# rrwick/Badread

Hardware: NVIDIA H100
Metric: simulated Gbases/sec (higher is better)
Workload: dtype u8/int32 (+f64 identity estimate)

## Files before the change

badread_b200/csrc/bb_api.cu:

```cuda
#include <cuda_runtime.h>
#include <dlfcn.h>
#include <unistd.h>

#include <algorithm>
#include <atomic>
#include <cstdio>
#include <cstdlib>
#include <cstring>
#include <numeric>
#include <string>
#include <thread>
#include <vector>

#include "bb_kernels.cuh"
#include "bb_launch.h"

namespace {

struct DevBuf {
    void *p = nullptr;
    size_t cap = 0;
    bool borrowed = false;
    void borrow(const DevBuf &o) { release(); p = o.p; cap = o.cap; borrowed = true; }
    cudaError_t ensure(size_t bytes) {
        if (bytes <= cap && !borrowed) return cudaSuccess;
        if (borrowed) { p = nullptr; cap = 0; borrowed = false; }
        if (p) { cudaFree(p); p = nullptr; cap = 0; }
        size_t want = bytes + bytes / 8 + 256;
        cudaError_t e = cudaMalloc(&p, want);
        if (e == cudaSuccess) cap = want;
        return e;
    }
    void release() { if (p && !borrowed) cudaFree(p); p = nullptr; cap = 0; borrowed = false; }
    template <typename T> T *as() const { return reinterpret_cast<T *>(p); }
};

constexpr int BB_MAX_ROUNDS = 15;

const char *kStageNames[BB_N_STAGES] = {"build_fragments", "error_loop", "scan", "join", "final_align", "qscores",
                                        "compact", "total"};

}

struct bb_ctx {
    int device = 0;
    int sm_count = 0;
    uint64_t seed = 0;
    cudaStream_t stream = nullptr, stream2 = nullptr;
    cudaStream_t side[2][3] = {};
    cudaEvent_t ev_side[2][3] = {}, ev_level[2] = {};
    cudaEvent_t ev_fork = nullptr, ev_join = nullptr;
    std::string err;
    int64_t launches = 0;

    DevBuf ref; int64_t ref_len = 0;
    bool have_em = false, have_qm = false;
    BBErrorModelDev em{}; DevBuf em_k2r, em_rowoff, em_cum, em_flags, em_slots, em_pool, em_rowinfo;
    BBQScoreModelDev qm{}; DevBuf qm_hkeys, qm_hvals, qm_lkeys, qm_lpool, qm_rowoff, qm_scores, qm_cum;

    int n_reads = 0;
    bool uploaded = false, ran = false;
    std::vector<BBReadDev> h_reads;
    std::vector<int32_t> h_inlen;
    std::vector<double> h_target;
    int64_t frag_total = 0, out_total = 0;
    int64_t seq_cap = 0, out_cap = 0, speq_cap = 0;
    int64_t log_total = 0, wres_total = 0;
    int max_len = 0;
    double slack = 1.25;
    int n_rounds = 3;
    int n_levels = 0;
    int extra_levels = 0;
    bool lr_worst = false;
    int lr_cap = 0;
    struct RunInfo { BBScanOut scan; int counters[256]; int qcount[2][32]; } *h_info = nullptr;
    std::vector<BBReadDev> h_res;
    bool finished = false;
    bool reran = false;
    int n_reruns = 0;
    uint32_t rerun_reasons = 0;
    DevBuf d_scan;
    void *nccl_comm = nullptr;
    DevBuf d_red;
    cudaEvent_t ev_scan = nullptr;
    DevBuf d_read_index, d_seg_off, d_segs, d_lit, d_target, d_order, d_reads;
    int n_lane_reads = 0, n_long_reads = 0;
    std::vector<int> h_order;
    DevBuf d_kidx, d_frag, d_state, d_seq, d_ops, d_dcnt, d_qual, d_out_seq, d_out_qual, d_counter, d_fpeq, d_speq, d_fallback;
    int64_t fpeq_total = 0;

    int n_warps = 0;
    BBScratchPool pool{}, pool_lean{};
    DevBuf s_hist, s_hbuf, s_lr, s_stack, s_tbuf, s_peq, s_ltbuf, s_leafhist, s_lr_lean, s_wckpt, s_lanehist;
    DevBuf d_ctime, d_chlog, d_wres, d_wtasks, d_wfallback, d_active;
    DevBuf p_q, p_t, p_ops, p_dcnt, p_out, p_qual;
    int lane8_cols = 4096;
    int pair_ctas = 1;
    bool head_worker = true;
    bool is_head = false;
    bool lpt_order = true;
    int ring_t = 4;
    bool lowmem = false;
    bool use_quad = false;
    int grid_div_env = 0;
    int grid_div = 1;
    struct QueueBufs { DevBuf node[BBQ_NODE_CLASSES][2], leaf[2], count; } qbuf[2];


    cudaEvent_t ev[BB_N_STAGES + 1] = {};
    float stage_ms[BB_N_STAGES] = {};

    std::vector<bb_ctx *> kids;
    int n_split = 1;
    std::vector<std::vector<int32_t>> part;
    std::vector<int64_t> part_base;
    cudaEvent_t ev_t0 = nullptr, ev_t1 = nullptr;

    bool trace = false;
    struct Mark { const char *name; int stream; cudaEvent_t ev; };
    std::vector<Mark> marks;
    std::vector<cudaEvent_t> mark_pool;
    size_t mark_used = 0;
};

static void mark(bb_ctx *ctx, cudaStream_t st, const char *name) {
    if (!ctx->trace) return;
    if (ctx->mark_used == ctx->mark_pool.size()) {
        cudaEvent_t e;
        if (cudaEventCreate(&e) != cudaSuccess) return;
        ctx->mark_pool.push_back(e);
    }
    cudaEvent_t e = ctx->mark_pool[ctx->mark_used++];
    cudaEventRecord(e, st);
    int id = st == ctx->stream ? 0 : st == ctx->stream2 ? 1 : -1;
    for (int p = 0; p < 2 && id < 0; p++)
        for (int x = 0; x < 3; x++)
            if (st == ctx->side[p][x]) id = 2 + 4 * p + x;
    ctx->marks.push_back(bb_ctx::Mark{name, id < 0 ? 0 : id, e});
}

static thread_local std::string g_create_error;

namespace {
struct ConnectionsDefault {
    ConnectionsDefault() { setenv("CUDA_DEVICE_MAX_CONNECTIONS", "32", 0); }
} g_connections_default;
}

#define BB_CUDA(ctx, call)                                                                                   \
    do {                                                                                                     \
        cudaError_t e_ = (call);                                                                             \
        if (e_ != cudaSuccess) {                                                                             \
            (ctx)->err = std::string(#call) + ": " + cudaGetErrorString(e_);                                 \
            return BB_ERR_CUDA;                                                                              \
        }                                                                                                    \
    } while (0)

static int set_err(bb_ctx *ctx, int code, const std::string &msg) {
    if (ctx) ctx->err = msg;
    return code;
}

extern "C" const char *bb_version(void) { return "badread_b200 0.1.0 (sm_90a)"; }

extern "C" const char *bb_last_error(const bb_ctx *ctx) { return ctx ? ctx->err.c_str() : g_create_error.c_str(); }

extern "C" const char *bb_stage_name(int stage) {
    return (stage >= 0 && stage < BB_N_STAGES) ? kStageNames[stage] : "";
}

extern "C" int64_t bb_launch_count(const bb_ctx *ctx) {
    if (!ctx) return 0;
    int64_t total = ctx->launches;
    for (const bb_ctx *kid : ctx->kids) total += kid->launches;
    return total;
}

static int create_worker(bb_ctx **out, int device, uint64_t seed, bool high_priority = false) {
    if (!out) return BB_ERR_ARG;
    *out = nullptr;
    int n_dev = 0;
    cudaError_t e = cudaGetDeviceCount(&n_dev);
    if (e != cudaSuccess || n_dev <= 0) {
        g_create_error = std::string("no CUDA device available: ") + cudaGetErrorString(e) +
                         " (badread_b200 has no CPU path)";
        return BB_ERR_CUDA;
    }
    if (device < 0 || device >= n_dev) { g_create_error = "invalid device ordinal"; return BB_ERR_ARG; }
    e = cudaSetDevice(device);
    if (e != cudaSuccess) { g_create_error = cudaGetErrorString(e); return BB_ERR_CUDA; }
    bb_ctx *ctx = new bb_ctx();
    ctx->device = device;
    ctx->seed = seed;
    cudaDeviceProp prop;
    e = cudaGetDeviceProperties(&prop, device);
    if (e != cudaSuccess) { g_create_error = cudaGetErrorString(e); delete ctx; return BB_ERR_CUDA; }
    ctx->sm_count = prop.multiProcessorCount;
    int prio_lo = 0, prio_hi = 0;
    cudaDeviceGetStreamPriorityRange(&prio_lo, &prio_hi);
    const int prio = high_priority ? prio_hi : prio_lo;
    e = cudaStreamCreateWithPriority(&ctx->stream, cudaStreamNonBlocking, prio);
    if (e != cudaSuccess) { g_create_error = cudaGetErrorString(e); delete ctx; return BB_ERR_CUDA; }
    for (auto &ev : ctx->ev) cudaEventCreate(&ev);
    cudaStreamCreateWithPriority(&ctx->stream2, cudaStreamNonBlocking, prio);
    cudaEventCreateWithFlags(&ctx->ev_fork, cudaEventDisableTiming);
    cudaEventCreateWithFlags(&ctx->ev_join, cudaEventDisableTiming);
    cudaEventCreateWithFlags(&ctx->ev_scan, cudaEventDisableTiming);
    for (int p = 0; p < 2; p++) {
        cudaEventCreateWithFlags(&ctx->ev_level[p], cudaEventDisableTiming);
        for (int x = 0; x < 3; x++) {
            cudaStreamCreateWithPriority(&ctx->side[p][x], cudaStreamNonBlocking, prio);
            cudaEventCreateWithFlags(&ctx->ev_side[p][x], cudaEventDisableTiming);
        }
    }
    if (cudaHostAlloc((void **)&ctx->h_info, sizeof(bb_ctx::RunInfo), cudaHostAllocPortable) != cudaSuccess) {
        g_create_error = "cudaHostAlloc failed"; delete ctx; return BB_ERR_CUDA;
    }
    uint8_t comp[256];
    std::memset(comp, 'N', sizeof(comp));
    const char *from = "ATGCatgcRYSWKMBVDHNryswkmbvdhn.-?";
    const char *to = "TACGtacgYRSWMKVBHDNyrswmkvbhdn.-?";
    for (int i = 0; from[i]; i++) comp[(uint8_t)from[i]] = (uint8_t)to[i];
    e = cudaMemcpyToSymbol(bb_c_comp, comp, 256);
    if (e != cudaSuccess) { g_create_error = cudaGetErrorString(e); delete ctx; return BB_ERR_CUDA; }
    e = bbl_node_pair_init();
    if (e == cudaSuccess) e = bbl_node_quad_init();
    if (e == cudaSuccess) e = bbl_window_lane_init();
    if (e == cudaSuccess) e = bbl_leaf_lane_init();
    if (e != cudaSuccess) { g_create_error = cudaGetErrorString(e); delete ctx; return BB_ERR_CUDA; }
    ctx->n_warps = ctx->sm_count * 4 * BB_WARPS_PER_CTA;
    if (const char *e = std::getenv("BADREAD_B200_TRACE")) ctx->trace = (e[0] == '1');
    if (const char *e = std::getenv("BADREAD_B200_LANE8_COLS")) ctx->lane8_cols = std::atoi(e);
    if (const char *e = std::getenv("BADREAD_B200_PAIR_CTAS")) ctx->pair_ctas = (e[0] == '2') ? 2 : 1;
    if (const char *e = std::getenv("BADREAD_B200_HEAD_WORKER")) ctx->head_worker = (e[0] != '0');
    if (const char *e = std::getenv("BADREAD_B200_GRID_DIV")) ctx->grid_div_env = std::atoi(e);
    if (const char *e = std::getenv("BADREAD_B200_QUAD")) ctx->use_quad = (e[0] != '0');
    if (const char *e = std::getenv("BADREAD_B200_LOWMEM")) ctx->lowmem = (e[0] != '0');
    if (const char *e = std::getenv("BADREAD_B200_LPT")) ctx->lpt_order = (e[0] != '0');
    if (const char *e = std::getenv("BADREAD_B200_RING_T")) ctx->ring_t = (e[0] == '8') ? 8 : (e[0] == '2') ? 2 : 4;
    if (const char *e = std::getenv("BADREAD_B200_ROUNDS")) ctx->n_rounds = std::max(1, std::min(BB_MAX_ROUNDS, std::atoi(e)));
    if (const char *e = std::getenv("BADREAD_B200_SLACK")) { const double v = std::atof(e); if (v > 0.0) ctx->slack = v; }
    if (const char *e = std::getenv("BADREAD_B200_EXTRA_LEVELS")) ctx->extra_levels = std::atoi(e);
    if (const char *e = std::getenv("BADREAD_B200_LR_CAP")) ctx->lr_cap = std::max(0, std::atoi(e));
    *out = ctx;
    return BB_OK;
}

extern "C" int bb_destroy(bb_ctx *ctx);
static void (*nccl_destroy)(void *) = nullptr;

extern "C" int bb_create(bb_ctx **out, int device, uint64_t seed) {
    bool prio = true;
    if (const char *e = std::getenv("BADREAD_B200_HEAD_PRIORITY")) prio = (e[0] != '0');
    int rc = create_worker(out, device, seed, prio);
    if (rc) return rc;
    bb_ctx *ctx = *out;
    int n_workers = 2;
    if (const char *e = std::getenv("BADREAD_B200_SUBBATCHES")) n_workers = std::max(1, std::min(8, std::atoi(e)));
    for (int w = 1; w < n_workers; w++) {
        bb_ctx *kid = nullptr;
        if ((rc = create_worker(&kid, device, seed))) { bb_destroy(ctx); *out = nullptr; return rc; }
        ctx->kids.push_back(kid);
    }
    cudaEventCreate(&ctx->ev_t0);
    cudaEventCreate(&ctx->ev_t1);
    return BB_OK;
}

extern "C" int bb_destroy(bb_ctx *ctx) {
    if (!ctx) return BB_OK;
    for (bb_ctx *kid : ctx->kids) bb_destroy(kid);
    ctx->kids.clear();
    cudaSetDevice(ctx->device);
    cudaStreamSynchronize(ctx->stream);
    if (ctx->ev_t0) cudaEventDestroy(ctx->ev_t0);
    if (ctx->ev_t1) cudaEventDestroy(ctx->ev_t1);
    DevBuf *bufs[] = {&ctx->ref, &ctx->em_k2r, &ctx->em_rowoff, &ctx->em_cum, &ctx->em_flags, &ctx->em_slots,
                      &ctx->em_pool, &ctx->em_rowinfo, &ctx->qm_hkeys, &ctx->qm_hvals, &ctx->qm_lkeys, &ctx->qm_lpool, &ctx->qm_rowoff, &ctx->qm_scores, &ctx->qm_cum,
                      &ctx->d_read_index, &ctx->d_seg_off, &ctx->d_segs, &ctx->d_lit, &ctx->d_target, &ctx->d_order,
                      &ctx->d_reads, &ctx->d_kidx, &ctx->d_frag, &ctx->d_state, &ctx->d_seq, &ctx->d_ops, &ctx->d_dcnt,
                      &ctx->d_qual, &ctx->d_out_seq, &ctx->d_out_qual, &ctx->d_counter, &ctx->s_hist, &ctx->s_hbuf,
                      &ctx->s_lr, &ctx->s_stack, &ctx->s_tbuf, &ctx->s_peq, &ctx->s_ltbuf, &ctx->d_ctime, &ctx->d_chlog, &ctx->d_wres,
                      &ctx->d_wtasks, &ctx->d_wfallback, &ctx->d_active,
                      &ctx->d_fpeq, &ctx->d_speq, &ctx->d_fallback, &ctx->s_leafhist, &ctx->s_lr_lean, &ctx->s_wckpt, &ctx->s_lanehist, &ctx->d_scan, &ctx->d_red,
                      &ctx->p_q, &ctx->p_t, &ctx->p_ops, &ctx->p_dcnt, &ctx->p_out, &ctx->p_qual};
    for (auto &qb : ctx->qbuf) {
        for (auto &cl : qb.node) for (auto &d : cl) d.release();
        qb.leaf[0].release(); qb.leaf[1].release(); qb.count.release();
    }
    for (DevBuf *b : bufs) b->release();
    for (auto &ev : ctx->ev) if (ev) cudaEventDestroy(ev);
    cudaStreamDestroy(ctx->stream);
    if (ctx->stream2) cudaStreamDestroy(ctx->stream2);
    if (ctx->ev_fork) cudaEventDestroy(ctx->ev_fork);
    if (ctx->ev_join) cudaEventDestroy(ctx->ev_join);
    if (ctx->ev_scan) cudaEventDestroy(ctx->ev_scan);
    for (int p = 0; p < 2; p++) {
        if (ctx->ev_level[p]) cudaEventDestroy(ctx->ev_level[p]);
        for (int x = 0; x < 3; x++) {
            if (ctx->side[p][x]) cudaStreamDestroy(ctx->side[p][x]);
            if (ctx->ev_side[p][x]) cudaEventDestroy(ctx->ev_side[p][x]);
        }
    }
    if (ctx->h_info) cudaFreeHost(ctx->h_info);
    if (ctx->nccl_comm && nccl_destroy) nccl_destroy(ctx->nccl_comm);
    for (cudaEvent_t e : ctx->mark_pool) cudaEventDestroy(e);
    delete ctx;
    return BB_OK;
}

template <typename T>
static int upload(bb_ctx *ctx, DevBuf &buf, const T *src, size_t count) {
    BB_CUDA(ctx, buf.ensure(std::max<size_t>(count, 1) * sizeof(T)));
    if (count) BB_CUDA(ctx, cudaMemcpyAsync(buf.p, src, count * sizeof(T), cudaMemcpyHostToDevice, ctx->stream));
    return BB_OK;
}

extern "C" int bb_upload_reference(bb_ctx *ctx, const uint8_t *bases, int64_t n_bases) {
    if (!ctx || n_bases < 0 || (n_bases && !bases)) return set_err(ctx, BB_ERR_ARG, "bb_upload_reference: bad arguments");
    BB_CUDA(ctx, cudaSetDevice(ctx->device));
    int rc = upload(ctx, ctx->ref, bases, (size_t)n_bases);
    if (rc) return rc;
    BB_CUDA(ctx, cudaStreamSynchronize(ctx->stream));
    ctx->ref_len = n_bases;
    for (bb_ctx *kid : ctx->kids) { kid->ref.borrow(ctx->ref); kid->ref_len = n_bases; }
    return BB_OK;
}

extern "C" int bb_upload_error_model(bb_ctx *ctx, int k, int type, const int32_t *kmer_to_row, int64_t n_index,
                                     int32_t n_rows, const int32_t *row_off, const double *cum, const uint8_t *flags,
                                     const uint32_t *slots, const uint8_t *pool, int64_t pool_len) {
    if (!ctx) return BB_ERR_ARG;
    if (k < 1 || k > 12 || (type != 0 && type != 1)) return set_err(ctx, BB_ERR_ARG, "error model: k must be 1..12");
    BB_CUDA(ctx, cudaSetDevice(ctx->device));
    ctx->em = BBErrorModelDev{};
    ctx->em.k = k; ctx->em.type = type;
    if (type == 1) {
        if (!kmer_to_row || !row_off || !cum || !flags || !slots || n_rows <= 0 || n_index != (1ll << (2 * k)))
            return set_err(ctx, BB_ERR_ARG, "error model: missing tables");
        const int64_t ne = row_off[n_rows];
        int rc;
        if ((rc = upload(ctx, ctx->em_k2r, kmer_to_row, (size_t)n_index))) return rc;
        if ((rc = upload(ctx, ctx->em_rowoff, row_off, (size_t)n_rows + 1))) return rc;
        if ((rc = upload(ctx, ctx->em_cum, cum, (size_t)ne))) return rc;
        if ((rc = upload(ctx, ctx->em_flags, flags, (size_t)ne))) return rc;
        if ((rc = upload(ctx, ctx->em_slots, slots, (size_t)ne * k))) return rc;
        if ((rc = upload(ctx, ctx->em_pool, pool, (size_t)pool_len))) return rc;
        std::vector<BBRowInfo> info((size_t)n_rows);
        for (int32_t r = 0; r < n_rows; r++) {
            const int32_t e0 = row_off[r], ne = row_off[r + 1] - e0;
            if (ne <= 0) return set_err(ctx, BB_ERR_ARG, "error model: empty table row");
            BBRowInfo &ri = info[(size_t)r];
// ... 289 lines not shown
                                 ctx->s_lanehist.as<uint2>(), ctx->s_ltbuf.as<uint8_t>(), c + BBC_LANE8, fb2, c + BBC_FB2);
        mark(ctx, st, "window_lane8");
        bbl_window_warp(pgrid(ctx, 2), st, B, ctx->em, ctx->pool, fb2, c + BBC_FB2, ctx->seed, c + BBC_WARP);
        mark(ctx, st, "window_warp");
        bb_k_replay<<<(n + 3) / 4, 128, 0, st>>>(B, order, n, ctx->em.k, c + BBC_PENDING);
        mark(ctx, st, "replay");
        ctx->launches += 6;
    }
    return BB_OK;
}

static int enqueue_align_tasks(bb_ctx *ctx, const BBBatchDev &B) {
    cudaStream_t stream[2] = {ctx->stream, ctx->stream2};
    const int n = ctx->n_reads;
    const int cap_node = (int)std::min<int64_t>(ctx->seq_cap / 256 + 4ll * n + 1024, 0x7ffffff0);
    const int lane_ctas = ctx->sm_count * 4;
    const size_t hist_per_pipe = (size_t)lane_ctas * 64 * BB_LEAF_MAX_TILES * BB_LEAF_CKPT_WORDS;
    BBQueues Q[2];
    int *cnt[2];
    for (int s = 0; s < 2; s++) {
        auto &qb = ctx->qbuf[s];
        for (int c = 0; c < BBQ_NODE_CLASSES; c++)
            for (int p = 0; p < 2; p++) Q[s].node[c][p] = qb.node[c][p].as<BBNode>();
        for (int w = 0; w < 2; w++) Q[s].leaf[w] = qb.leaf[w].as<BBNode>();
        cnt[s] = qb.count.as<int>();
        Q[s].count = cnt[s]; Q[s].overflow = cnt[s] + BBQ_OVERFLOW; Q[s].cap_node = cap_node; Q[s].cap_leaf = cap_node;
        Q[s].lane8_cols = ctx->lane8_cols;
        BB_CUDA(ctx, cudaMemsetAsync(cnt[s], 0, 512 * sizeof(int), stream[0]));
    }
    bb_k_push_roots<<<(n + 255) / 256, 256, 0, stream[0]>>>(B, Q[0], Q[1], ctx->d_order.as<int>());
    ctx->launches++;
    BB_CUDA(ctx, cudaEventRecord(ctx->ev_fork, stream[0]));
    BB_CUDA(ctx, cudaStreamWaitEvent(stream[1], ctx->ev_fork, 0));
    int *cursor[2] = {cnt[0] + 16, cnt[1] + 16};
    const int warp_base[2] = {0, ctx->n_warps / 2};
    const int w4 = ctx->sm_count * 4 * BB_WARPS_PER_CTA, w2 = ctx->sm_count * 6 * BB_WARPS_PER_CTA;
    const int lean_base[2] = {0, w4 + 2 * w2};
    for (int level = 0; level < ctx->n_levels; level++) {
        const int p = (level & 1) | (level > 0 && ctx->lpt_order ? BBQ_BACKWARDS : 0);
        for (int s = 0; s < 2; s++) {
            cudaStream_t st = stream[s];
            BB_CUDA(ctx, cudaMemsetAsync(cnt[s] + BBQ_COUNT(0, (p & 1) ^ 1), 0, BBQ_NODE_CLASSES * sizeof(int), st));
            BB_CUDA(ctx, cudaEventRecord(ctx->ev_level[s], st));
            int n_side = 0;
            auto on_side = [&]() -> cudaStream_t {
                cudaStream_t x = ctx->side[s][n_side++];
                cudaStreamWaitEvent(x, ctx->ev_level[s], 0);
                mark(ctx, x, "fork");
                return x;
            };
            if (s == 1) {
                cudaStream_t x = on_side();
                if (ctx->use_quad) bbl_node_quad(ctx->sm_count, x, B, Q[s], ctx->pool, p, cursor[s]++, warp_base[s]);
                else bbl_node_pair(ctx->sm_count * ctx->pair_ctas, x, B, Q[s], ctx->pool, p, cursor[s]++, warp_base[s]);
                ctx->launches++;
                mark(ctx, x, ctx->use_quad ? "node_quad" : "node_pair");
            }
            {
                cudaStream_t x = on_side();
                bbl_node_warp(2, std::min(pgrid(ctx, 3, "WARP2"), ctx->sm_count * 6), x, B, Q[s], ctx->pool_lean, p, cursor[s]++, lean_base[s] + w4);
                mark(ctx, x, "node_warp2");
                bbl_node_warp(1, std::min(pgrid(ctx, 3, "WARP1"), ctx->sm_count * 6), x, B, Q[s], ctx->pool_lean, p, cursor[s]++, lean_base[s] + w4 + w2);
                mark(ctx, x, "node_warp1");
                x = on_side();
                bbl_node_lane8(pgrid(ctx, 6, "LANE8"), x, B, Q[s], p, cursor[s]++);
                mark(ctx, x, "node_lane8");
            }
            bbl_node_warp(4, std::min(pgrid(ctx, 2, "WARP4"), ctx->sm_count * 4), st, B, Q[s], ctx->pool_lean, p, cursor[s]++, lean_base[s]);
            mark(ctx, st, "node_warp4");
            ctx->launches += 4;
            for (int x = 0; x < n_side; x++) {
                BB_CUDA(ctx, cudaEventRecord(ctx->ev_side[s][x], ctx->side[s][x]));
                BB_CUDA(ctx, cudaStreamWaitEvent(st, ctx->ev_side[s][x], 0));
            }
        }
    }
    for (int s = 0; s < 2; s++) {
        cudaStream_t st = stream[s];
        bbl_leaf_warp(ctx->sm_count, st, B, Q[s], ctx->pool, cursor[s]++, warp_base[s]);
        mark(ctx, st, "leaf_warp");
        if (ctx->lowmem)
            bbl_leaf_lane(std::min(pgrid(ctx, 3, "LEAF"), ctx->sm_count * 4), st, B, Q[s], ctx->s_leafhist.as<uint32_t>() + s * hist_per_pipe, cursor[s]++);
        else
            bbl_leaf_lane_hist(std::min(pgrid(ctx, 4, "LEAF"), ctx->sm_count * 4), st, B, Q[s],
                               ctx->s_lanehist.as<uint2>() + s * ((size_t)lane_ctas * 64 * BB_LEAF_LANE_COLS * BB_LEAF_LW), cursor[s]++);
        mark(ctx, st, "leaf_lane");
        ctx->launches += 2;
    }
    BB_CUDA(ctx, cudaEventRecord(ctx->ev_join, stream[1]));
    BB_CUDA(ctx, cudaStreamWaitEvent(stream[0], ctx->ev_join, 0));
    for (int s = 0; s < 2; s++)
        BB_CUDA(ctx, cudaMemcpyAsync(ctx->h_info->qcount[s], cnt[s], 32 * sizeof(int), cudaMemcpyDeviceToHost, stream[0]));
    return BB_OK;
}

static int w_enqueue(bb_ctx *ctx) {
    if (!ctx) return BB_ERR_ARG;
    if (!ctx->uploaded) return set_err(ctx, BB_ERR_STATE, "bb_batch_run: no batch uploaded");
    BB_CUDA(ctx, cudaSetDevice(ctx->device));
    cudaStream_t st = ctx->stream;
    const int n = ctx->n_reads;
    BBBatchDev B = batch_dev(ctx);
    ctx->finished = false;
    BB_CUDA(ctx, cudaMemcpyAsync(ctx->d_reads.p, ctx->h_reads.data(), (size_t)n * sizeof(BBReadDev), cudaMemcpyHostToDevice, st));
    BB_CUDA(ctx, cudaMemsetAsync(ctx->d_counter.p, 0, BB_N_COUNTERS * sizeof(int), st));
    ctx->marks.clear(); ctx->mark_used = 0;
    mark(ctx, st, "begin");
// ... 602 lines not shown
```

badread_b200/csrc/bb_launch.h:

```cpp
#pragma once
#include <cuda_runtime.h>

#include "bb_kernels.cuh"

void bbl_mutate(int grid, cudaStream_t st, BBBatchDev B, BBErrorModelDev em, unsigned long long seed, int *work_counter,
                const int *order, int n_items, bool chain);
cudaError_t bbl_window_lane_init();
void bbl_window_lane4(int grid, cudaStream_t st, BBBatchDev B, BBErrorModelDev em, const BBWinTask *tasks, const int *n_tasks,
                      unsigned long long seed, uint32_t *ckpt_pool, uint8_t *tbuf_pool, int *cursor, BBWinTask *fallback,
                      int *fallback_count);
void bbl_window_lane8(int grid, cudaStream_t st, BBBatchDev B, BBErrorModelDev em, const BBWinTask *tasks, const int *n_tasks,
                      unsigned long long seed, uint32_t *ckpt_pool, uint8_t *tbuf_pool, int *cursor, BBWinTask *fallback,
                      int *fallback_count);
void bbl_window_lane_hist(int words, int ring_t, int grid, cudaStream_t st, BBBatchDev B, BBErrorModelDev em, const BBWinTask *tasks,
                          const int *n_tasks, unsigned long long seed, uint2 *hist_pool, uint8_t *tbuf_pool, int *cursor,
                          BBWinTask *fallback, int *fallback_count);
void bbl_window_warp(int grid, cudaStream_t st, BBBatchDev B, BBErrorModelDev em, BBScratchPool pool, const BBWinTask *tasks,
                     const int *n_tasks, unsigned long long seed, int *cursor);
void bbl_node_warp(int words, int grid, cudaStream_t st, BBBatchDev B, BBQueues Q, BBScratchPool pool, int parity, int *cursor,
                   int warp_base);
void bbl_node_lane8(int grid, cudaStream_t st, BBBatchDev B, BBQueues Q, int parity, int *cursor);
cudaError_t bbl_node_quad_init();
void bbl_node_quad(int grid, cudaStream_t st, BBBatchDev B, BBQueues Q, BBScratchPool pool, int parity, int *cursor,
                   int warp_base);
cudaError_t bbl_node_pair_init();
void bbl_node_pair(int grid, cudaStream_t st, BBBatchDev B, BBQueues Q, BBScratchPool pool, int parity, int *cursor,
                   int warp_base);
void bbl_leaf_warp(int grid, cudaStream_t st, BBBatchDev B, BBQueues Q, BBScratchPool pool, int *cursor, int warp_base);
void bbl_leaf_lane_hist(int grid, cudaStream_t st, BBBatchDev B, BBQueues Q, uint2 *hist_pool, int *cursor);
cudaError_t bbl_leaf_lane_init();
void bbl_leaf_lane(int grid, cudaStream_t st, BBBatchDev B, BBQueues Q, uint32_t *ckpt_pool, int *cursor);
void bbl_align_pair(cudaStream_t st, const uint8_t *q, int n, const uint8_t *t, int m, int k_upper, BBScratchPool pool,
                    uint8_t *ops, unsigned int *dcnt, int *out5);
```

badread_b200/csrc/bb_tasks.cuh:

```cuda
#pragma once
#include <cstdint>

#include "bb_align.cuh"
#include "bb_lane.cuh"

#define BB_NODE_LW_SMALL 8
#define BB_LEAF_LW 8
#define BB_LEAF_LANE_COLS 2048

enum { BBQ_NODE_LANE8 = 0, BBQ_NODE_LEAN1 = 1, BBQ_NODE_LEAN2 = 2, BBQ_NODE_LEAN4 = 3, BBQ_NODE_WIDE = 4, BBQ_NODE_CLASSES = 5 };
#define BBQ_COUNT(cls, parity) ((parity) * BBQ_NODE_CLASSES + (cls))
#define BBQ_LEAF_COUNT 10
#define BBQ_OVERFLOW 12
#define BBQ_BACKWARDS 2

struct BBNode { int r, q0, nn, t0, mm, best; };

struct BBQueues {
    BBNode *node[BBQ_NODE_CLASSES][2];
    BBNode *leaf[2];
    int *count;
    int *overflow;
    int cap_node, cap_leaf;
    int lane8_cols;
};

struct BBAlignOut {
    uint8_t *ops;
    unsigned int *dcnt;
    BBReadDev *rd;
};

__device__ __forceinline__ void bb_add_dels(const BBAlignOut &o, int qidx_after, int count) {
    if (count <= 0) return;
    if (qidx_after >= 0) atomicAdd(&o.dcnt[qidx_after], (unsigned int)count);
    else atomicAdd(&o.rd->lead_del, count);
}

__device__ __forceinline__ void bb_task_band(const BBNode &nd, int upper, int &a, int &b) {
    int k = nd.best >= 0 ? nd.best : upper;
    const int diff = nd.nn > nd.mm ? nd.nn - nd.mm : nd.mm - nd.nn;
    if (k < diff) k = diff;
    const int mx = nd.nn > nd.mm ? nd.nn : nd.mm;
    if (k > mx) k = mx;
    bb_band(nd.nn, nd.mm, k, a, b);
    a += a & 1; b += b & 1;
}

static __device__ void bb_push_task(const BBQueues &Q, int next_parity, const BBAlignOut &o, const BBNode &nd, int upper) {
    if (nd.nn == 0) {
        atomicAdd(&o.rd->dels, nd.mm);
        bb_add_dels(o, nd.q0 - 1, nd.mm);
        return;
    }
    if (nd.mm == 0) {
        for (int x = 0; x < nd.nn; x++) o.ops[nd.q0 + x] = BB_OP_I;
        return;
    }
    int a, b;
    bb_task_band(nd, upper, a, b);
    const int lw = bb_lane_words(a, b);
    if (bb_uses_traceback(nd.nn, nd.mm)) {
        const int which = (lw <= BB_LEAF_LW && nd.mm <= BB_LEAF_LANE_COLS) ? 0 : 1;
        const int idx = atomicAdd(&Q.count[BBQ_LEAF_COUNT + which], 1);
        if (idx >= Q.cap_leaf) { atomicExch(Q.overflow, 1); return; }
        Q.leaf[which][idx] = nd;
    } else {
// ... 114 lines not shown
        S.Pv[x] = mhs | ~(Xv[x] | phs);
        S.Mv[x] = phs & Xv[x];
        if (HIST && (HSTRIDE != 1 || (LW & 1))) hist[x * HSTRIDE] = make_uint2(S.Pv[x], raw);
        if (HIST && HSTRIDE == 1 && !(LW & 1)) Ph[x] = raw;
    }
    if (HIST && HSTRIDE == 1 && !(LW & 1)) {
#pragma unroll
        for (int x = 0; x < LW; x += 2)
            reinterpret_cast<uint4 *>(hist)[x >> 1] = make_uint4(S.Pv[x], Ph[x], S.Pv[x + 1], Ph[x + 1]);
    }
    S.c = c + 1;
}

template <int LW>
__device__ int bb_lane_column_scores(const BBLanePass<LW> &S, int n, int lo, int hi, int *out) {
    int result = BB_INF;
    int run = S.score;
#pragma unroll
    for (int x = LW - 1; x >= 0; x--) {
        const int row0 = (S.wt + x) * 32;
        int rr = run;
        for (int r = 31; r >= 0; r--) {
            const int row = row0 + r;
            if (row < n) {
                if (out && row >= lo && row <= hi) out[row - lo] = rr;
                if (row == n - 1) result = rr;
            }
            rr -= (int)((S.Pv[x] >> r) & 1u) - (int)((S.Mv[x] >> r) & 1u);
        }
        run -= __popc(S.Pv[x]) - __popc(S.Mv[x]);
    }
    return result;
}

template <int LW>
__device__ __forceinline__ int bb_lane_corner(const BBLanePass<LW> &S, int n) {
    int result = BB_INF;
    int run = S.score;
#pragma unroll
    for (int x = LW - 1; x >= 0; x--) {
        const int row0 = (S.wt + x) * 32;
        if (row0 <= n - 1 && n - 1 < row0 + 32) {
            const int bit = (n - 1) - row0;
            const uint32_t up = bit == 31 ? 0u : (S.Pv[x] >> (bit + 1));
            const uint32_t um = bit == 31 ? 0u : (S.Mv[x] >> (bit + 1));
            result = run - __popc(up) + __popc(um);
        }
        run -= __popc(S.Pv[x]) - __popc(S.Mv[x]);
    }
    return result;
}

template <int LW>
__global__ void __launch_bounds__(64, 6)
bb_k_node_lane(BBBatchDev B, BBQueues Q, int parity_order, int *cursor) {
    constexpr int CLS = BBQ_NODE_LANE8;
    const int parity = parity_order & 1;
    const bool backwards = (parity_order & BBQ_BACKWARDS) != 0;
    const BBNode *list = Q.node[CLS][parity];
    const int count = min(Q.count[BBQ_COUNT(CLS, parity)], Q.cap_node);
    BBLanePass<LW> S;
    BBProb P;
    BBNode nd;
    int Lc[32 * LW], Rc[32 * LW];
    int loL = 0, hiL = 0, loR = 0, hiR = 0, left_w = 0, right_w = 0, ncols = 0, upper = 0;
    int phase = 0;
    BBAlignOut o;
    for (;;) {
        if (phase == 0) {
            const int w = atomicAdd(cursor, 1);
            if (w >= count) phase = 3;
            else {
                nd = list[backwards ? count - 1 - w : w];
                BBReadDev *rd = &B.reads[nd.r];
                o.ops = B.ops + rd->seq_off; o.dcnt = B.dcnt + rd->seq_off; o.rd = rd;
                upper = rd->upper;
                bb_task_band(nd, upper, P.a, P.b);
                left_w = nd.mm / 2; right_w = nd.mm - left_w;
                loL = max(0, left_w - 1 - P.a); hiL = min(nd.nn - 1, left_w - 1 + P.b);
                loR = max(0, right_w - 1 - P.a); hiR = min(nd.nn - 1, right_w - 1 + P.b);
                P.n = nd.nn; P.peq = B.speq + rd->speq_off;
                P.q = B.seq + rd->seq_off + nd.q0; P.qs = 1; P.peq_bit0 = nd.q0 + BB_PEQ_BIT0;
                P.t = B.frag + rd->frag_off + nd.t0; P.ts = 1;
                ncols = left_w;
                bb_lane_begin<LW>(S, P);
                phase = 1;
            }
        }
        if (__all_sync(BB_FULL, phase == 3)) break;
        for (int it = 0; it < 128; it++) {
            if (phase == 1 || phase == 2) {
                bb_lane_step<LW, false>(S, P, nullptr);
                if (S.c >= ncols) {
                    if (phase == 1) {
                        bb_lane_column_scores<LW>(S, nd.nn, loL, hiL, Lc);
                        const BBReadDev *rd = o.rd;
                        P.q = B.seq + rd->seq_off + nd.q0 + nd.nn - 1; P.qs = -1; P.peq_bit0 = nd.q0 + nd.nn - 1 + BB_PEQ_BIT0;
                        P.t = B.frag + rd->frag_off + nd.t0 + nd.mm - 1; P.ts = -1;
                        ncols = right_w;
                        bb_lane_begin<LW>(S, P);
                        phase = 2;
                    } else {
                        bb_lane_column_scores<LW>(S, nd.nn, loR, hiR, Rc);
                        int best = nd.best, split = 0, ls = 0, rs = 0;
                        if (!bb_choose_split_seq(Lc, loL, hiL, Rc, loR, hiR, nd.nn, left_w, right_w, best, split, ls, rs)) {
                            atomicOr(&o.rd->flags, 32 << 8);
                        } else {
                            BBNode c0 = {nd.r, nd.q0, split + 1, nd.t0, left_w, ls};
                            BBNode c1 = {nd.r, nd.q0 + split + 1, nd.nn - split - 1, nd.t0 + left_w, right_w, rs};
                            bb_push_task(Q, parity ^ 1, o, c0, upper);
                            bb_push_task(Q, parity ^ 1, o, c1, upper);
                        }
                        phase = 0;
                    }
                }
            }
        }
    }
}

#define BB_LEAF_TILE 16
#define BB_LEAF_CKPT_WORDS (2 * BB_LEAF_LW + 2)
#define BB_LEAF_MAX_TILES (BB_LEAF_LANE_COLS / BB_LEAF_TILE)
#define BB_LEAF_SMEM_BYTES (BB_LEAF_TILE * BB_LEAF_LW * 64 * 8)

template <int BB_TU_ = 0>
__global__ void __launch_bounds__(64, 3)
bb_k_leaf_lane(BBBatchDev B, BBQueues Q, uint32_t *ckpt_pool, int *cursor) {
    constexpr int LW = BB_LEAF_LW, CKW = BB_LEAF_CKPT_WORDS;
#ifdef BB_EMULATOR
    static uint2 s_hist[BB_LEAF_TILE * LW * 64];
#else
    extern __shared__ __align__(16) uint2 s_hist[];
#endif
    const BBNode *list = Q.leaf[0];
    const int count = min(Q.count[BBQ_LEAF_COUNT], Q.cap_leaf);
    uint32_t *const ckpt = ckpt_pool + ((long long)blockIdx.x * blockDim.x + threadIdx.x) * (long long)(BB_LEAF_MAX_TILES * CKW);
    uint2 *const hs = s_hist + threadIdx.x;
    for (;;) {
        const int w = atomicAdd(cursor, 1);
        const bool active = w < count;
        if (!__any_sync(BB_FULL, active)) break;
        BBNode nd = {0, 0, 0, 0, 0, 0};
        BBAlignOut o = {nullptr, nullptr, nullptr};
        BBProb P;
        P.a = 0; P.b = 1;
        BBLanePass<LW> S;
        const uint8_t *qp = nullptr, *tp = nullptr;
        int mm = 0;
        if (active) {
            nd = list[w];
            BBReadDev *rd = &B.reads[nd.r];
            o.ops = B.ops + rd->seq_off; o.dcnt = B.dcnt + rd->seq_off; o.rd = rd;
            bb_task_band(nd, rd->upper, P.a, P.b);
            P.n = nd.nn; P.peq = B.speq + rd->speq_off;
            qp = B.seq + rd->seq_off + nd.q0; tp = B.frag + rd->frag_off + nd.t0;
            P.q = qp; P.qs = 1; P.peq_bit0 = nd.q0 + BB_PEQ_BIT0; P.t = tp; P.ts = 1;
            bb_lane_begin<LW>(S, P);
// ... 103 lines not shown
                bb_task_band(nd, rd->upper, P.a, P.b);
                P.n = nd.nn; P.peq = B.speq + rd->speq_off;
                qp = B.seq + rd->seq_off + nd.q0; tp = B.frag + rd->frag_off + nd.t0;
                P.q = qp; P.qs = 1; P.peq_bit0 = nd.q0 + BB_PEQ_BIT0; P.t = tp; P.ts = 1;
                bb_lane_begin<LW>(S, P);
                phase = 1;
            }
        }
        if (__all_sync(BB_FULL, phase == 3)) break;
        for (int it = 0; it < 128; it++) {
            if (phase == 1) {
                bb_lane_step<LW, true>(S, P, hist + (long long)S.c * LW);
                if (S.c >= nd.mm) {
                    const int d = bb_lane_corner<LW>(S, nd.nn);
                    if (nd.best >= 0 && d != nd.best) atomicOr(&o.rd->flags, 8 << 8);
                    ti = nd.nn - 1; tj = nd.mm - 1; matches = 0; dels = 0; staged_lo = nd.mm;
                    phase = 2;
                }
            }
        }
        for (int it = 0; it < 256; it++) {
            if (phase == 2) {
                if (ti >= 0 && tj >= 0) {
                    if ((it & (T - 1)) == 0) bb_ring_tick<LW, T>(ring, hist, tj, staged_lo);
                    int wt = (tj - P.a) >> 5; if (wt < 0) wt = 0;
                    const int x = (ti >> 5) - wt;
                    if (x < 0 || x >= LW) { atomicOr(&o.rd->flags, 1 << 8); ti = -1; tj = -1; }
                    else {
                        const uint2 e = bb_ring_entry<LW, T>(ring, tj, x);
                        const int bit = ti & 31;
                        if ((e.x >> bit) & 1u) { o.ops[nd.q0 + ti] = BB_OP_I; ti--; }
                        else if ((e.y >> bit) & 1u) { bb_add_dels(o, nd.q0 + ti, 1); dels++; tj--; }
                        else {
                            const bool eq = qp[ti] == tp[tj];
                            o.ops[nd.q0 + ti] = eq ? BB_OP_EQ : BB_OP_X;
                            matches += eq ? 1 : 0;
                            ti--; tj--;
                        }
                    }
                } else {
                    bb_cp_async_wait<0>();
                    for (int x = 0; x <= ti; x++) o.ops[nd.q0 + x] = BB_OP_I;
                    if (tj >= 0) { bb_add_dels(o, nd.q0 - 1, tj + 1); dels += tj + 1; }
                    atomicAdd(&o.rd->matches, matches);
                    atomicAdd(&o.rd->dels, dels);
                    phase = 0;
                }
            }
        }
    }
}

template <int L>
__global__ void __launch_bounds__(BB_WARPS_PER_CTA * 32, (L == 1 ? 6 : L == 2 ? 5 : 3))
bb_k_node_warp(BBBatchDev B, BBQueues Q, BBScratchPool pool, int parity_order, int *cursor, int warp_base) {
    constexpr int CLS = L == 1 ? BBQ_NODE_LEAN1 : L == 2 ? BBQ_NODE_LEAN2 : BBQ_NODE_LEAN4;
    const int parity = parity_order & 1;
    const bool backwards = (parity_order & BBQ_BACKWARDS) != 0;
    const int lane = threadIdx.x & 31;
    const int warp = warp_base + blockIdx.x * BB_WARPS_PER_CTA + (threadIdx.x >> 5);
    BBScratch sc = pool.for_warp(warp);
    const BBNode *list = Q.node[CLS][parity];
    const int count = min(Q.count[BBQ_COUNT(CLS, parity)], Q.cap_node);
    for (;;) {
        int w = 0;
        if (lane == 0) w = atomicAdd(cursor, 1);
        w = __shfl_sync(BB_FULL, w, 0);
        if (w >= count) break;
        const BBNode nd = list[backwards ? count - 1 - w : w];
        BBReadDev *rd = &B.reads[nd.r];
        BBAlignOut o;
        o.ops = B.ops + rd->seq_off; o.dcnt = B.dcnt + rd->seq_off; o.rd = rd;
        sc.peq = B.speq + rd->speq_off;
        const uint8_t *q = B.seq + rd->seq_off, *t = B.frag + rd->frag_off;
        int a, b;
        bb_task_band(nd, rd->upper, a, b);
        const int left_w = nd.mm / 2, right_w = nd.mm - left_w;
        const int loL = max(0, left_w - 1 - a), hiL = min(nd.nn - 1, left_w - 1 + b);
        const int loR = max(0, right_w - 1 - a), hiR = min(nd.nn - 1, right_w - 1 + b);
        int best = nd.best, split = 0, ls = 0, rs = 0, err = 0;
        if (hiL - loL + 1 > sc.lr_cap || hiR - loR + 1 > sc.lr_cap) err = 16;
        else {
            BBProb P;
            P.n = nd.nn; P.a = a; P.b = b; P.peq = sc.peq; P.hist = nullptr; P.nb_alloc = 0;
            P.tpeq = B.fpeq + rd->fpeq_off;
            if (lane < 16) {
                P.q = q + nd.q0; P.qs = 1; P.t = t + nd.t0; P.ts = 1; P.ncols = left_w;
                P.peq_bit0 = nd.q0 + BB_PEQ_BIT0; P.cols_out = sc.L; P.cols_lo = loL;
                P.tpeq_bit0 = nd.t0 + BB_PEQ_BIT0;
            } else {
                P.q = q + nd.q0 + nd.nn - 1; P.qs = -1; P.t = t + nd.t0 + nd.mm - 1; P.ts = -1; P.ncols = right_w;
                P.peq_bit0 = nd.q0 + nd.nn - 1 + BB_PEQ_BIT0; P.cols_out = sc.R; P.cols_lo = loR;
                P.tpeq_bit0 = nd.t0 + nd.mm - 1 + BB_PEQ_BIT0;
            }
            bb_band_pass_bp<L>(P, 16);
            __syncwarp();
            err = bb_split_warp(sc, loL, hiL, loR, hiR, nd.nn, left_w, right_w, best, split, ls, rs);
        }
        __syncwarp();
        if (lane == 0) {
            if (err) atomicOr(&rd->flags, err << 8);
            else {
                BBNode c0 = {nd.r, nd.q0, split + 1, nd.t0, left_w, ls};
                BBNode c1 = {nd.r, nd.q0 + split + 1, nd.nn - split - 1, nd.t0 + left_w, right_w, rs};
                bb_push_task(Q, parity ^ 1, o, c0, rd->upper);
                bb_push_task(Q, parity ^ 1, o, c1, rd->upper);
            }
        }
        __syncwarp();
    }
}

#define BB_PAIR_SMEM_BYTES (BB_WARPS_PER_CTA * bb_esm_words(32) * 4)

__device__ __forceinline__ void bb_pair_sync(int id) {
#ifdef BB_EMULATOR
    emu::named_barrier(id, 64);
#else
    asm volatile("bar.sync %0, 64;" ::"r"(id) : "memory");
#endif
}

template <int BB_TU_ = 0>
__global__ void __launch_bounds__(BB_WARPS_PER_CTA * 32, 2)
bb_k_node_pair(BBBatchDev B, BBQueues Q, BBScratchPool pool, int parity_order, int *cursor, int warp_base) {
    const int parity = parity_order & 1;
    const bool backwards = (parity_order & BBQ_BACKWARDS) != 0;
    __shared__ int s_task[BB_WARPS_PER_CTA / 2];
#ifdef BB_EMULATOR
    static uint32_t s_eq[BB_PAIR_SMEM_BYTES / 4];
#else
    extern __shared__ __align__(16) uint32_t s_eq[];
#endif
    const int lane = threadIdx.x & 31;
    const int wi = threadIdx.x >> 5;
    const int pair = wi >> 1;
    const bool rev = (wi & 1) != 0;
    BBScratch sc = pool.for_warp(warp_base + blockIdx.x * BB_WARPS_PER_CTA + (wi & ~1));
    const BBNode *list = Q.node[BBQ_NODE_WIDE][parity];
    const int count = min(Q.count[BBQ_COUNT(BBQ_NODE_WIDE, parity)], Q.cap_node);
    for (;;) {
        if (!rev && lane == 0) s_task[pair] = atomicAdd(cursor, 1);
        bb_pair_sync(pair + 1);
        const int w = s_task[pair];
        bb_pair_sync(pair + 1);
        if (w >= count) break;
        const BBNode nd = list[backwards ? count - 1 - w : w];
        BBReadDev *rd = &B.reads[nd.r];
        sc.peq = B.speq + rd->speq_off;
        const uint8_t *q = B.seq + rd->seq_off, *t = B.frag + rd->frag_off;
        int a, b;
        bb_task_band(nd, rd->upper, a, b);
        const int left_w = nd.mm / 2, right_w = nd.mm - left_w;
        const int loL = max(0, left_w - 1 - a), hiL = min(nd.nn - 1, left_w - 1 + b);
        const int loR = max(0, right_w - 1 - a), hiR = min(nd.nn - 1, right_w - 1 + b);
        const int L = bb_pick_L<32>(a, b, 32);
        int err = 0;
        if (hiL - loL + 1 > sc.lr_cap || hiR - loR + 1 > sc.lr_cap) err = 16;
        else if (L > 0) {
            BBProb P;
            P.n = nd.nn; P.a = a; P.b = b; P.peq = sc.peq; P.hist = nullptr; P.nb_alloc = 0;
            if (!rev) {
                P.q = q + nd.q0; P.qs = 1; P.t = t + nd.t0; P.ts = 1; P.ncols = left_w;
                P.peq_bit0 = nd.q0 + BB_PEQ_BIT0; P.cols_out = sc.L; P.cols_lo = loL;
            } else {
                P.q = q + nd.q0 + nd.nn - 1; P.qs = -1; P.t = t + nd.t0 + nd.mm - 1; P.ts = -1; P.ncols = right_w;
                P.peq_bit0 = nd.q0 + nd.nn - 1 + BB_PEQ_BIT0; P.cols_out = sc.R; P.cols_lo = loR;
            }
            P.esm = s_eq + wi * bb_esm_words(32);
            bb_band_dispatch<false, true, 32, true>(P, 32, L);
        }
        __threadfence_block();
        bb_pair_sync(pair + 1);
        if (!rev) {
            int best = nd.best, split = 0, ls = 0, rs = 0;
            if (!err) {
                if (L > 0) err = bb_split_warp(sc, loL, hiL, loR, hiR, nd.nn, left_w, right_w, best, split, ls, rs);
                else err = bb_node_warp<1>(q, t, nd.q0, nd.nn, nd.t0, nd.mm, a, b, sc, best, split, ls, rs);
            }
            if (lane == 0) {
                BBAlignOut o;
                o.ops = B.ops + rd->seq_off; o.dcnt = B.dcnt + rd->seq_off; o.rd = rd;
                if (err) atomicOr(&rd->flags, err << 8);
                else {
                    BBNode c0 = {nd.r, nd.q0, split + 1, nd.t0, left_w, ls};
                    BBNode c1 = {nd.r, nd.q0 + split + 1, nd.nn - split - 1, nd.t0 + left_w, right_w, rs};
                    bb_push_task(Q, parity ^ 1, o, c0, rd->upper);
                    bb_push_task(Q, parity ^ 1, o, c1, rd->upper);
                }
            }
            __syncwarp();
        }
    }
}

#define BB_QUAD_WARPS 4
#define BB_QUAD_THREADS (2 * BB_QUAD_WARPS * 32)
#define BB_QUAD_SMEM_BYTES (2 * BB_QUAD_WARPS * bb_esm_words(32) * 4)

template <int BB_TU_ = 0>
__global__ void __launch_bounds__(BB_QUAD_THREADS, 1)
bb_k_node_quad(BBBatchDev B, BBQueues Q, BBScratchPool pool, int parity_order, int *cursor, int warp_base) {
    const int parity = parity_order & 1;
    const bool backwards = (parity_order & BBQ_BACKWARDS) != 0;
    __shared__ int s_task;
    __shared__ uint32_t s_mbox[2][BB_QUAD_WARPS * 8];
    __shared__ int s_progress[2][BB_QUAD_WARPS];
    __shared__ int s_err;
#ifdef BB_EMULATOR
    static uint32_t s_eq[BB_QUAD_SMEM_BYTES / 4];
#else
    extern __shared__ __align__(16) uint32_t s_eq[];
#endif
    const int lane = threadIdx.x & 31;
    const int wi = threadIdx.x >> 5;
    const bool rev = wi >= BB_QUAD_WARPS;
    const int wg = wi % BB_QUAD_WARPS;
    BBScratch sc = pool.for_warp(warp_base + blockIdx.x);
    const BBNode *list = Q.node[BBQ_NODE_WIDE][parity];
    const int count = min(Q.count[BBQ_COUNT(BBQ_NODE_WIDE, parity)], Q.cap_node);
    for (;;) {
        if (threadIdx.x == 0) { s_task = atomicAdd(cursor, 1); s_err = 0; }
        if (threadIdx.x < 2 * BB_QUAD_WARPS) s_progress[threadIdx.x / BB_QUAD_WARPS][threadIdx.x % BB_QUAD_WARPS] = 0;
        __syncthreads();
        const int w = s_task;
        __syncthreads();
        if (w >= count) break;
        const BBNode nd = list[backwards ? count - 1 - w : w];
        BBReadDev *rd = &B.reads[nd.r];
        sc.peq = B.speq + rd->speq_off;
        const uint8_t *q = B.seq + rd->seq_off, *t = B.frag + rd->frag_off;
// ... 94 lines not shown
```

badread_b200/csrc/bb_tu_node_pair.cu:

```cuda
#include "bb_launch.h"

cudaError_t bbl_node_pair_init() {
    return cudaFuncSetAttribute(bb_k_node_pair<0>, cudaFuncAttributeMaxDynamicSharedMemorySize, BB_PAIR_SMEM_BYTES);
}

void bbl_node_pair(int grid, cudaStream_t st, BBBatchDev B, BBQueues Q, BBScratchPool pool, int parity, int *cursor,
                   int warp_base) {
    bb_k_node_pair<0><<<grid, BB_WARPS_PER_CTA * 32, BB_PAIR_SMEM_BYTES, st>>>(B, Q, pool, parity, cursor, warp_base);
}
```

Measured before the change: 1.104.

## Split node-pair by band width, compute lane splits from bit-vectors, tweak bounds

```diff
diff --git a/badread_b200/csrc/bb_api.cu b/badread_b200/csrc/bb_api.cu
--- a/badread_b200/csrc/bb_api.cu
+++ b/badread_b200/csrc/bb_api.cu
@@ -47,8 +47,8 @@
     int sm_count = 0;
     uint64_t seed = 0;
     cudaStream_t stream = nullptr, stream2 = nullptr;
-    cudaStream_t side[2][3] = {};
-    cudaEvent_t ev_side[2][3] = {}, ev_level[2] = {};
+    cudaStream_t side[2][4] = {};
+    cudaEvent_t ev_side[2][4] = {}, ev_level[2] = {};
     cudaEvent_t ev_fork = nullptr, ev_join = nullptr;
     std::string err;
     int64_t launches = 0;
@@ -134,7 +134,7 @@
     cudaEventRecord(e, st);
     int id = st == ctx->stream ? 0 : st == ctx->stream2 ? 1 : -1;
     for (int p = 0; p < 2 && id < 0; p++)
-        for (int x = 0; x < 3; x++)
+        for (int x = 0; x < 4; x++)
             if (st == ctx->side[p][x]) id = 2 + 4 * p + x;
     ctx->marks.push_back(bb_ctx::Mark{name, id < 0 ? 0 : id, e});
 }
@@ -208,7 +208,7 @@
     cudaEventCreateWithFlags(&ctx->ev_scan, cudaEventDisableTiming);
     for (int p = 0; p < 2; p++) {
         cudaEventCreateWithFlags(&ctx->ev_level[p], cudaEventDisableTiming);
-        for (int x = 0; x < 3; x++) {
+        for (int x = 0; x < 4; x++) {
             cudaStreamCreateWithPriority(&ctx->side[p][x], cudaStreamNonBlocking, prio);
             cudaEventCreateWithFlags(&ctx->ev_side[p][x], cudaEventDisableTiming);
         }
@@ -297,7 +297,7 @@
     if (ctx->ev_scan) cudaEventDestroy(ctx->ev_scan);
     for (int p = 0; p < 2; p++) {
         if (ctx->ev_level[p]) cudaEventDestroy(ctx->ev_level[p]);
-        for (int x = 0; x < 3; x++) {
+        for (int x = 0; x < 4; x++) {
             if (ctx->side[p][x]) cudaStreamDestroy(ctx->side[p][x]);
             if (ctx->ev_side[p][x]) cudaEventDestroy(ctx->ev_side[p][x]);
         }
@@ -693,7 +693,15 @@
             if (s == 1) {
                 cudaStream_t x = on_side();
                 if (ctx->use_quad) bbl_node_quad(ctx->sm_count, x, B, Q[s], ctx->pool, p, cursor[s]++, warp_base[s]);
-                else bbl_node_pair(ctx->sm_count * ctx->pair_ctas, x, B, Q[s], ctx->pool, p, cursor[s]++, warp_base[s]);
+                else if (ctx->pair_ctas != 1)
+                    bbl_node_pair(ctx->sm_count * ctx->pair_ctas, x, B, Q[s], ctx->pool, p, cursor[s]++, warp_base[s], 0);
+                else {
+                    bbl_node_pair(ctx->sm_count, x, B, Q[s], ctx->pool, p, cursor[s]++, warp_base[s], 1);
+                    mark(ctx, x, "node_pair");
+                    x = on_side();
+                    bbl_node_pair(ctx->sm_count, x, B, Q[s], ctx->pool, p, cursor[s]++, warp_base[s] + ctx->sm_count * BB_WARPS_PER_CTA, 2);
+                    ctx->launches++;
+                }
                 ctx->launches++;
                 mark(ctx, x, ctx->use_quad ? "node_quad" : "node_pair");
             }
diff --git a/badread_b200/csrc/bb_launch.h b/badread_b200/csrc/bb_launch.h
--- a/badread_b200/csrc/bb_launch.h
+++ b/badread_b200/csrc/bb_launch.h
@@ -25,7 +25,8 @@
                    int warp_base);
 cudaError_t bbl_node_pair_init();
 void bbl_node_pair(int grid, cudaStream_t st, BBBatchDev B, BBQueues Q, BBScratchPool pool, int parity, int *cursor,
-                   int warp_base);
+                   int warp_base,
+                   int widths);
 void bbl_leaf_warp(int grid, cudaStream_t st, BBBatchDev B, BBQueues Q, BBScratchPool pool, int *cursor, int warp_base);
 void bbl_leaf_lane_hist(int grid, cudaStream_t st, BBBatchDev B, BBQueues Q, uint2 *hist_pool, int *cursor);
 cudaError_t bbl_leaf_lane_init();
diff --git a/badread_b200/csrc/bb_tasks.cuh b/badread_b200/csrc/bb_tasks.cuh
--- a/badread_b200/csrc/bb_tasks.cuh
+++ b/badread_b200/csrc/bb_tasks.cuh
@@ -13,6 +13,12 @@
 #define BBQ_LEAF_COUNT 10
 #define BBQ_OVERFLOW 12
 #define BBQ_BACKWARDS 2
+
+#ifdef BB_EMULATOR
+#define BB_GRID_CONST
+#else
+#define BB_GRID_CONST __grid_constant__
+#endif
 
 struct BBNode { int r, q0, nn, t0, mm, best; };
 
@@ -233,8 +239,112 @@
 }
 
 template <int LW>
+__device__ __forceinline__ int bb_lane_row_score(const uint32_t (&Pv)[LW], const uint32_t (&Mv)[LW], int wt, int score, int row) {
+    int v = score;
+#pragma unroll
+    for (int x = 0; x < LW; x++) {
+        const int k = row - (wt + x) * 32;
+        const uint32_t below = k < 0 ? ~0u : k >= 31 ? 0u : ~0u << (k + 1);
+        v -= __popc(Pv[x] & below) - __popc(Mv[x] & below);
+    }
+    return v;
+}
+
+template <int LW>
+__device__ __forceinline__ void bb_shift_rev_words(const uint32_t (&W)[LW], int e, uint32_t (&out)[LW + 1]) {
+    constexpr int M = LW + 1;
+#pragma unroll
+    for (int y = 0; y < M; y++) out[y] = y < LW ? W[LW - 1 - y] : 0u;
+    if (e >= M || e <= -M) {
+#pragma unroll
+        for (int y = 0; y < M; y++) out[y] = 0u;
+    }
+    const int left = e > 0 ? e : 0, right = e < 0 ? -e : 0;
+#pragma unroll
+    for (int b = 1; b < M; b <<= 1) {
+        if (left & b) {
+#pragma unroll
+            for (int y = 0; y < M; y++) out[y] = y + b < M ? out[y + b] : 0u;
+        }
+        if (right & b) {
+#pragma unroll
+            for (int y = M - 1; y >= 0; y--) out[y] = y - b >= 0 ? out[y - b] : 0u;
+        }
+    }
+}
+
+template <int LW>
+__device__ __forceinline__ bool bb_lane_split(const uint32_t (&FP)[LW], const uint32_t (&FM)[LW], int fwt, int fscore,
+                                              const uint32_t (&RP)[LW], const uint32_t (&RM)[LW], int rwt, int rscore,
+                                              int loL, int hiL, int loR, int hiR, int nn, int left_w, int right_w,
+                                              int &best, int &split, int &ls, int &rs) {
+    int rlo = max(loL, nn - 2 - hiR); if (rlo < 0) rlo = 0;
+    int rhi = min(hiL, nn - 2 - loR); if (rhi > nn - 2) rhi = nn - 2;
+    const bool have_top = nn - 1 >= loR && nn - 1 <= hiR;
+    const bool have_bot = nn - 1 >= loL && nn - 1 <= hiL;
+    const bool root = best < 0;
+    const int off = nn - 32 - 32 * (fwt + rwt);
+    const int k0 = off >> 5, sh = off & 31;
+    uint32_t HP[LW + 1], HM[LW + 1];
+    bb_shift_rev_words<LW>(RP, LW - 2 - k0, HP);
+    bb_shift_rev_words<LW>(RM, LW - 2 - k0, HM);
+    uint32_t AP[LW], AM[LW];
+    int S0[LW], up[LW], dn[LW];
+    int s = bb_lane_row_score<LW>(FP, FM, fwt, fscore, 32 * fwt - 1) + bb_lane_row_score<LW>(RP, RM, rwt, rscore, nn - 1 - 32 * fwt);
+#pragma unroll
+    for (int x = 0; x < LW; x++) {
+        AP[x] = __brev(__funnelshift_r(HP[x + 1], HP[x], sh));
+        AM[x] = __brev(__funnelshift_r(HM[x + 1], HM[x], sh));
+        S0[x] = s;
+        up[x] = __popc(FP[x]) + __popc(AM[x]);
+        dn[x] = __popc(FM[x]) + __popc(AP[x]);
+        s += up[x] - dn[x];
+    }
+    int mn = BB_INF, at = -1;
+    for (int done = -1; done < LW - 1;) {
+        int pick = -1, sv = 0;
+        uint32_t fp = 0u, fm = 0u, ap = 0u, am = 0u;
+#pragma unroll
+        for (int x = LW - 1; x >= 0; x--) {
+            const int r0 = 32 * (fwt + x);
+            const bool can = x > done && r0 <= rhi && r0 + 31 >= rlo &&
+                             (root ? S0[x] - dn[x] < mn : S0[x] - dn[x] <= best && best <= S0[x] + up[x]);
+            if (can) { pick = x; sv = S0[x]; fp = FP[x]; fm = FM[x]; ap = AP[x]; am = AM[x]; }
+        }
+        if (pick < 0) break;
+        done = pick;
+        const int r0 = 32 * (fwt + pick);
+        bool found = false;
+        for (int i = 0; i < 32; i++) {
+            sv += (int)((fp >> i) & 1u) - (int)((fm >> i) & 1u) - (int)((ap >> i) & 1u) + (int)((am >> i) & 1u);
+            const int r = r0 + i;
+            if (r >= rlo && r <= rhi && (root ? sv < mn : sv == best)) {
+                mn = sv; at = r;
+                if (!root) { found = true; break; }
+            }
+        }
+        if (found) break;
+    }
+    const int top = have_top ? left_w + bb_lane_row_score<LW>(RP, RM, rwt, rscore, nn - 1) : BB_INF;
+    const int bot = have_bot ? bb_lane_row_score<LW>(FP, FM, fwt, fscore, nn - 1) + right_w : BB_INF;
+    if (root) {
+        best = min(mn, min(top, bot));
+        if (mn != best) at = -1;
+    }
+    if (at >= 0) {
+        split = at;
+        ls = bb_lane_row_score<LW>(FP, FM, fwt, fscore, at);
+        rs = bb_lane_row_score<LW>(RP, RM, rwt, rscore, nn - 2 - at);
+        return true;
+    }
+    if (have_top && top == best) { split = -1; ls = left_w; rs = top - left_w; return true; }
+    if (have_bot && bot == best) { split = nn - 1; ls = bot - right_w; rs = right_w; return true; }
+    return false;
+}
+
+template <int LW>
 __global__ void __launch_bounds__(64, 6)
-bb_k_node_lane(BBBatchDev B, BBQueues Q, int parity_order, int *cursor) {
+bb_k_node_lane(BBBatchDev B, const BB_GRID_CONST BBQueues Q, int parity_order, int *cursor) {
     constexpr int CLS = BBQ_NODE_LANE8;
     const int parity = parity_order & 1;
     const bool backwards = (parity_order & BBQ_BACKWARDS) != 0;
@@ -243,7 +353,8 @@
     BBLanePass<LW> S;
     BBProb P;
     BBNode nd;
-    int Lc[32 * LW], Rc[32 * LW];
+    uint32_t FP[LW], FM[LW];
+    int fwt = 0, fscore = 0;
     int loL = 0, hiL = 0, loR = 0, hiR = 0, left_w = 0, right_w = 0, ncols = 0, upper = 0;
     int phase = 0;
     BBAlignOut o;
@@ -274,7 +385,9 @@
                 bb_lane_step<LW, false>(S, P, nullptr);
                 if (S.c >= ncols) {
                     if (phase == 1) {
-                        bb_lane_column_scores<LW>(S, nd.nn, loL, hiL, Lc);
+#pragma unroll
+                        for (int x = 0; x < LW; x++) { FP[x] = S.Pv[x]; FM[x] = S.Mv[x]; }
+                        fwt = S.wt; fscore = S.score;
                         const BBReadDev *rd = o.rd;
                         P.q = B.seq + rd->seq_off + nd.q0 + nd.nn - 1; P.qs = -1; P.peq_bit0 = nd.q0 + nd.nn - 1 + BB_PEQ_BIT0;
                         P.t = B.frag + rd->frag_off + nd.t0 + nd.mm - 1; P.ts = -1;
@@ -282,9 +395,9 @@
                         bb_lane_begin<LW>(S, P);
                         phase = 2;
                     } else {
-                        bb_lane_column_scores<LW>(S, nd.nn, loR, hiR, Rc);
                         int best = nd.best, split = 0, ls = 0, rs = 0;
-                        if (!bb_choose_split_seq(Lc, loL, hiL, Rc, loR, hiR, nd.nn, left_w, right_w, best, split, ls, rs)) {
+                        if (!bb_lane_split<LW>(FP, FM, fwt, fscore, S.Pv, S.Mv, S.wt, S.score, loL, hiL, loR, hiR, nd.nn, left_w,
+                                               right_w, best, split, ls, rs)) {
                             atomicOr(&o.rd->flags, 32 << 8);
                         } else {
                             BBNode c0 = {nd.r, nd.q0, split + 1, nd.t0, left_w, ls};
@@ -494,8 +607,8 @@
 }
 
 template <int L>
-__global__ void __launch_bounds__(BB_WARPS_PER_CTA * 32, (L == 1 ? 6 : L == 2 ? 5 : 3))
-bb_k_node_warp(BBBatchDev B, BBQueues Q, BBScratchPool pool, int parity_order, int *cursor, int warp_base) {
+__global__ void __launch_bounds__(BB_WARPS_PER_CTA * 32, (L == 1 ? 4 : L == 2 ? 4 : 3))
+bb_k_node_warp(BBBatchDev B, const BB_GRID_CONST BBQueues Q, BBScratchPool pool, int parity_order, int *cursor, int warp_base) {
     constexpr int CLS = L == 1 ? BBQ_NODE_LEAN1 : L == 2 ? BBQ_NODE_LEAN2 : BBQ_NODE_LEAN4;
     const int parity = parity_order & 1;
     const bool backwards = (parity_order & BBQ_BACKWARDS) != 0;
@@ -563,7 +676,7 @@
 #endif
 }
 
-template <int BB_TU_ = 0>
+template <int BB_TU_ = 0, int LMIN = 1, int LMAX = 32>
 __global__ void __launch_bounds__(BB_WARPS_PER_CTA * 32, 2)
 bb_k_node_pair(BBBatchDev B, BBQueues Q, BBScratchPool pool, int parity_order, int *cursor, int warp_base) {
     const int parity = parity_order & 1;
@@ -597,6 +710,7 @@
         const int loL = max(0, left_w - 1 - a), hiL = min(nd.nn - 1, left_w - 1 + b);
         const int loR = max(0, right_w - 1 - a), hiR = min(nd.nn - 1, right_w - 1 + b);
         const int L = bb_pick_L<32>(a, b, 32);
+        if (L == 0 ? LMAX < 32 : (L < LMIN || L > LMAX)) continue;
         int err = 0;
         if (hiL - loL + 1 > sc.lr_cap || hiR - loR + 1 > sc.lr_cap) err = 16;
         else if (L > 0) {
@@ -610,7 +724,12 @@
                 P.peq_bit0 = nd.q0 + nd.nn - 1 + BB_PEQ_BIT0; P.cols_out = sc.R; P.cols_lo = loR;
             }
             P.esm = s_eq + wi * bb_esm_words(32);
-            bb_band_dispatch<false, true, 32, true>(P, 32, L);
+            if (LMIN >= 16) {
+                if (LMAX >= 32 && L == 32) bb_band_pass<(LMAX >= 32 ? 32 : 16), false, true, true>(P, 32);
+                else bb_band_pass<16, false, true, true>(P, 32);
+            } else {
+                bb_band_dispatch<false, true, LMAX, true>(P, 32, L);
+            }
         }
         __threadfence_block();
         bb_pair_sync(pair + 1);
@@ -618,7 +737,7 @@
             int best = nd.best, split = 0, ls = 0, rs = 0;
             if (!err) {
                 if (L > 0) err = bb_split_warp(sc, loL, hiL, loR, hiR, nd.nn, left_w, right_w, best, split, ls, rs);
-                else err = bb_node_warp<1>(q, t, nd.q0, nd.nn, nd.t0, nd.mm, a, b, sc, best, split, ls, rs);
+                else if (LMAX >= 32) err = bb_node_warp<1>(q, t, nd.q0, nd.nn, nd.t0, nd.mm, a, b, sc, best, split, ls, rs);
             }
             if (lane == 0) {
                 BBAlignOut o;
diff --git a/badread_b200/csrc/bb_tu_node_pair.cu b/badread_b200/csrc/bb_tu_node_pair.cu
--- a/badread_b200/csrc/bb_tu_node_pair.cu
+++ b/badread_b200/csrc/bb_tu_node_pair.cu
@@ -1,10 +1,20 @@
 #include "bb_launch.h"
 
 cudaError_t bbl_node_pair_init() {
-    return cudaFuncSetAttribute(bb_k_node_pair<0>, cudaFuncAttributeMaxDynamicSharedMemorySize, BB_PAIR_SMEM_BYTES);
+    cudaError_t e = cudaFuncSetAttribute(bb_k_node_pair<0>, cudaFuncAttributeMaxDynamicSharedMemorySize, BB_PAIR_SMEM_BYTES);
+    if (e == cudaSuccess)
+        e = cudaFuncSetAttribute(bb_k_node_pair<0, 1, 8>, cudaFuncAttributeMaxDynamicSharedMemorySize, BB_PAIR_SMEM_BYTES);
+    if (e == cudaSuccess)
+        e = cudaFuncSetAttribute(bb_k_node_pair<0, 16, 32>, cudaFuncAttributeMaxDynamicSharedMemorySize, BB_PAIR_SMEM_BYTES);
+    return e;
 }
 
 void bbl_node_pair(int grid, cudaStream_t st, BBBatchDev B, BBQueues Q, BBScratchPool pool, int parity, int *cursor,
-                   int warp_base) {
-    bb_k_node_pair<0><<<grid, BB_WARPS_PER_CTA * 32, BB_PAIR_SMEM_BYTES, st>>>(B, Q, pool, parity, cursor, warp_base);
+                   int warp_base, int widths) {
+    if (widths == 1)
+        bb_k_node_pair<0, 1, 8><<<grid, BB_WARPS_PER_CTA * 32, BB_PAIR_SMEM_BYTES, st>>>(B, Q, pool, parity, cursor, warp_base);
+    else if (widths == 2)
+        bb_k_node_pair<0, 16, 32><<<grid, BB_WARPS_PER_CTA * 32, BB_PAIR_SMEM_BYTES, st>>>(B, Q, pool, parity, cursor, warp_base);
+    else
+        bb_k_node_pair<0><<<grid, BB_WARPS_PER_CTA * 32, BB_PAIR_SMEM_BYTES, st>>>(B, Q, pool, parity, cursor, warp_base);
 }
```

After: 1.135 (median of 6 runs). 2.8% higher.
